# Easquel/WaveDM

Hardware: AMD Instinct MI355X
Metric: restored images/sec, raindrop 64x64 patches, 100-step DDIM (higher is better)
Workload: dtype bf16; 1 GPU; raindrop_wavelet 64x64 (256x256 px crops), batch 64/GPU, 100 DDIM steps, DWT + UNet x100 + IDWT (BASELINE.json configs[1]); global_batch=64, ddim_steps=100, parallelism=image-sharded x1, outputs_finite=True

## Files before the change

wavedm_amd/csrc/blocks.hip:

```cpp
#include <stdarg.h>

#include <algorithm>
#include <cmath>

#include <atomic>
#include <mutex>
#include "common.h"
#include "gn_inline.h"

namespace wdm {

static thread_local char g_err[512] = "";
void set_error(const char* fmt, ...) {
    va_list ap;
    va_start(ap, fmt);
    vsnprintf(g_err, sizeof(g_err), fmt, ap);
    va_end(ap);
}
const char* get_error() { return g_err; }

void* Arena::alloc(size_t bytes) {
    bytes = align_up(bytes ? bytes : 1, 256);
    for (size_t i = 0; i < free_.size(); ++i) {
        if (free_[i].len >= bytes) {
// ... 16 lines not shown
        if (used_[i].off == off) {
            Blk b = used_[i];
            used_.erase(used_.begin() + i);
            auto it = std::lower_bound(free_.begin(), free_.end(), b, [](const Blk& a, const Blk& c) { return a.off < c.off; });
            it = free_.insert(it, b);
            if (it + 1 != free_.end() && it->off + it->len == (it + 1)->off) { it->len += (it + 1)->len; free_.erase(it + 1); }
            if (it != free_.begin() && (it - 1)->off + (it - 1)->len == it->off) { (it - 1)->len += it->len; free_.erase(it); }
            return;
        }
    }
}

int alloc_tens(Ctx& c, int C, int H, int W, Tens* t) {
    *t = Tens();
    t->C = C; t->H = H; t->W = W; t->xs = C;
    t->p = c.ar->alloc((size_t)c.B * H * W * C * dsize(c.dtype));
    if (!t->p) WDM_FAIL(WDM_ENOMEM, "workspace too small (tensor %dx%dx%dx%d)", c.B, H, W, C);
    return WDM_OK;
}
void free_tens(Ctx& c, Tens& t) {
    c.ar->free(t.p);
    if (t.stats) c.ar->free(t.stats);
    if (t.nrm) c.ar->free(t.nrm);
    t.p = nullptr; t.stats = nullptr; t.gst = nullptr; t.nslab = 0; t.nrm = nullptr; t.nrm_for = nullptr;
}

static int alloc_f32(Ctx& c, size_t n, float** p) {
    *p = (float*)c.ar->alloc(n * sizeof(float));
    if (!*p) WDM_FAIL(WDM_ENOMEM, "workspace too small (%zu floats)", n);
    return WDM_OK;
}

static std::atomic<const EnvCfg*> g_env{nullptr};
static std::mutex g_env_mu;
void env_cfg_refresh() {
    EnvCfg* c = new EnvCfg();
    auto flag = [](const char* name, int dflt) { const char* e = getenv(name); return e ? (e[0] == '0' ? 0 : 1) : dflt; };
    auto num = [](const char* name, int dflt) { const char* e = getenv(name); return e ? atoi(e) : dflt; };
    c->conv_dma = flag("WDM_CONV_DMA", 1); c->gemm = flag("WDM_GEMM", 1); c->bn256 = num("WDM_BN256", 1);
    c->gn_tile = num("WDM_GN_TILE", 2); c->gn_inline = flag("WDM_GN_INLINE", 1); c->attn_fused = num("WDM_ATTN_FUSED", 3); c->attn_fold = num("WDM_ATTN_FOLD", 1);
    c->up4 = flag("WDM_UP4", 1); c->attn_sm = flag("WDM_ATTN_SM", 1); c->attn_stream = flag("WDM_ATTN_STREAM", 1); c->wgrad_bg = num("WDM_WGRAD_BG", 0);
    std::lock_guard<std::mutex> lk(g_env_mu);
    g_env.store(c, std::memory_order_release);
}
const EnvCfg& env_cfg() {
    const EnvCfg* c = g_env.load(std::memory_order_acquire);
    if (!c) {
        {
            std::lock_guard<std::mutex> lk(g_env_mu);
            c = g_env.load(std::memory_order_acquire);
        }
        if (!c) { env_cfg_refresh(); c = g_env.load(std::memory_order_acquire); }
    }
    return *c;
}

bool conv_up4_eligible(int dtype, int H, int W, int cin, int cout) {
    return env_cfg().up4 && (is_h16(dtype) || dtype == WDM_F32X3) && ((H % 16 == 0 && W % 16 == 0) || (H == 8 && W == 8)) && cin % 32 == 0 && cout % 8 == 0 && cout >= 128;
}

int launch_conv(const ConvArgs& a, int mode, int dtype, hipStream_t s) {
    return dtype == WDM_BF16 ? launch_conv_bf16(a, mode, s) : dtype == WDM_F16 ? launch_conv_f16(a, mode, s) : dtype == WDM_F32X3 ? launch_conv_f32x3(a, mode, s) : launch_conv_f32(a, mode, s);
}
ConvArgs gemm_args(int B, int H, int W, const void* x, int xs, int K, const void* w, int ws, long long w_img, int rows, int cout, void* y, int y_mode, size_t es,
                   float alpha) {
    ConvArgs a{};
    a.x0 = x; a.C0 = K; a.xs0 = xs;
    a.B = B; a.Hin = a.Hout = H; a.Win = a.Wout = W;
    a.Cin = K; a.Cout = cout;
    a.w = w; a.w_img_stride = w_img; a.w_row_stride = ws; a.w_rows = rows;
    a.w_bytes = (unsigned)((size_t)rows * ws * es);
    a.alpha = alpha;
    a.y = y; a.y_mode = y_mode; a.y_s = cout;
    return a;
}
int run_conv(Ctx& c, const ConvW& w, int mode, const ConvReq& r, Tens* out, ConvArgs* defer) {
    const Tens& x0 = *r.x0;
    const Tens* x1 = r.x1;
    const int Cin = x0.C + (x1 ? x1->C : 0);
    if (Cin != w.cin) WDM_FAIL(WDM_EINVAL, "conv: input has %d channels, weights expect %d", Cin, w.cin);
    if (x1 && (x1->H != x0.H || x1->W != x0.W)) WDM_FAIL(WDM_EINVAL, "conv: concat inputs differ in size");
    int Ho = x0.H, Wo = x0.W;
    if (mode == MODE_S2) { Ho = x0.H / 2; Wo = x0.W / 2; }
    if (mode == MODE_UPS) { Ho = x0.H * 2; Wo = x0.W * 2; }
    void* y = r.y_ext;
    const int y_mode = r.y_ext ? r.y_mode : Y_NHWC;
    if (!r.y_ext) {
        WDM_TRY(alloc_tens(c, w.cout, Ho, Wo, out));
        y = out->p;
    }
    ConvArgs a{};
    a.x0 = x0.p; a.x1 = x1 ? x1->p : nullptr;
    a.C0 = x0.C; a.C1 = x1 ? x1->C : 0;
    a.xs0 = x0.xs; a.xs1 = x1 ? x1->xs : 0;
    a.B = c.B; a.Hin = x0.H; a.Win = x0.W; a.Hout = Ho; a.Wout = Wo;
    a.Cin = Cin; a.Cout = w.cout;
    a.w = w.w; a.w_tap_stride = (long long)w.rows_pad * w.cin; a.w_img_stride = 0; a.w_row_stride = w.cin; a.w_rows = w.rows_pad;
    a.w_bytes = (unsigned)((size_t)w.k * w.k * w.rows_pad * w.cin * dsize(c.dtype));
    a.w_sm = ((mode == MODE_S1 || (mode == MODE_S2 && is_h16(c.dtype))) && w.k == 3) ? w.w_sm : nullptr;
    a.bias = w.b; a.alpha = 1.0f;
    a.pro = (r.scale || r.gn_inl) ? 1 : 0; a.scale = r.scale; a.shift = r.shift;
    if (r.gn_inl) {
        if (x1 || !x0.gst || r.scale || r.gn_inl->c != Cin) WDM_FAIL(WDM_EINVAL, "conv: in-prologue GroupNorm needs a single input with group partials");
        a.gin = x0.gst; a.gin_nslab = x0.nslab; a.gn_gamma = r.gn_inl->g; a.gn_beta = r.gn_inl->b; a.gn_eps = 1e-6f;
    }
    a.temb = r.temb; a.temb_ld = r.temb_ld; a.temb_per_image = r.temb_per_image;
    a.res = r.res ? r.res->p : nullptr; a.res_s = r.res ? r.res->xs : 0;
    a.y = y; a.y_mode = y_mode; a.y_s = w.cout;
    if (mode == MODE_UPS && w.w_up4 && !x1 && !r.scale && !r.temb && !r.res && !r.shortcut && y_mode == Y_NHWC && conv_up4_eligible(c.dtype, x0.H, x0.W, Cin, w.cout)) {
        mode = MODE_UP4;
        a.Hout = x0.H; a.Wout = x0.W;
        a.w = w.w_up4;
        a.w_bytes = (unsigned)((size_t)16 * w.rows_pad * w.cin * dsize(c.dtype));
    }
    if (r.shortcut) {
        a.sx0 = r.sx0->p; a.sx1 = r.sx1 ? r.sx1->p : nullptr;
        a.sC0 = r.sx0->C; a.sC1 = r.sx1 ? r.sx1->C : 0; a.sxs0 = r.sx0->xs; a.sxs1 = r.sx1 ? r.sx1->xs : 0;
        a.sw = r.shortcut->w; a.sw_row_stride = r.shortcut->cin; a.sw_rows = r.shortcut->rows_pad;
        a.sw_bytes = (unsigned)((size_t)r.shortcut->rows_pad * r.shortcut->cin * dsize(c.dtype));
        a.sbias = r.shortcut->b;
    }
    if (r.stats && !r.y_ext && w.cout % 8 == 0) {
        int nslab = 0, yn_ok = 0;
        ConvArgs q = a;
        q.query_nslab = &nslab; q.query_yn = &yn_ok;
        WDM_TRY(launch_conv(q, mode, c.dtype, c.s));
        out->nslab = nslab;
        if (r.on && yn_ok && env_cfg().gn_tile && r.on->c == w.cout) {
            out->nrm = c.ar->alloc((size_t)c.B * Ho * Wo * w.cout * dsize(c.dtype));
            if (!out->nrm) WDM_FAIL(WDM_ENOMEM, "workspace too small (normalised copy)");
            out->nrm_for = r.on->g; out->nrm_silu = r.on_silu;
            a.yn = out->nrm; a.on_gamma = r.on->g; a.on_beta = r.on->b; a.on_eps = 1e-6f; a.on_silu = r.on_silu;
        }
        const bool want_gst = is_h16(c.dtype) && env_cfg().gn_inline && gn_inline_shape_ok(w.cout, nslab);
        const size_t sb = gn_stats_bytes(c.B, nslab, w.cout);
        out->stats = (float*)c.ar->alloc(sb + (want_gst ? (size_t)c.B * nslab * 96 * sizeof(float) : 0));
        if (!out->stats) WDM_FAIL(WDM_ENOMEM, "workspace too small (GroupNorm statistics)");
        a.stats = out->stats; a.stats_nslab = nslab;
        if (want_gst) { out->gst = (float*)((char*)out->stats + sb); a.gst = out->gst; }
    }
    if (c.dry) return WDM_OK;
    if (defer) { *defer = a; return WDM_OK; }
    return launch_conv(a, mode, c.dtype, c.s);
}

static int gn_partials_of(Ctx& c, const Tens& x, float** st, int* ns, float** tmp) {
    *tmp = nullptr;
    if (x.stats) { *st = x.stats; *ns = x.nslab; return WDM_OK; }
    *ns = gn_default_nslab(x.H * x.W);
    *tmp = (float*)c.ar->alloc(gn_stats_bytes(c.B, *ns, x.C));
    if (!*tmp) WDM_FAIL(WDM_ENOMEM, "workspace too small (GroupNorm statistics)");
    *st = *tmp;
    if (!c.dry) WDM_TRY(k_gn_partial(x, c.B, *tmp, *ns, c.dtype, c.s));
    return WDM_OK;
}

int run_gn(Ctx& c, const NormW& nw, const Tens& x0, const Tens* x1, int for_silu_conv, float** scale, float** shift) {
    const int C = x0.C + (x1 ? x1->C : 0);
    WDM_TRY(alloc_f32(c, (size_t)c.B * C, scale));
    WDM_TRY(alloc_f32(c, (size_t)c.B * C, shift));
    float *st0 = nullptr, *st1 = nullptr, *tmp0 = nullptr, *tmp1 = nullptr;
    int ns0 = 0, ns1 = 0;
// ... 24 lines not shown
        int rc = WDM_OK;
        if (!c.dry) rc = k_gn_finalize_apply(c.B, x0, x1, st0, ns0, st1, ns1, nw, 1e-6f, silu, out->p, c.dtype, c.s);
        if (tmp0) c.ar->free(tmp0);
        if (tmp1) c.ar->free(tmp1);
        return rc;
    }
    float *sc, *sh;
    WDM_TRY(run_gn(c, nw, x0, x1, 0, &sc, &sh));
    WDM_TRY(alloc_tens(c, C, x0.H, x0.W, out));
    if (!c.dry) {
        WDM_TRY(k_gn_apply(x0, c.B, sc, sh, C, out->p, C, 0, silu, c.dtype, c.s));
        if (x1) WDM_TRY(k_gn_apply(*x1, c.B, sc + x0.C, sh + x0.C, C, out->p, C, x0.C, silu, c.dtype, c.s));
    }
    c.ar->free(sc); c.ar->free(sh);
    return WDM_OK;
}
static int materialize_gn_silu(Ctx& c, const NormW& nw, const Tens& x0, const Tens* x1, Tens* out) { return materialize_gn(c, nw, x0, x1, 1, out); }

static bool gn_inline_ok(const Ctx& c, const Tens& x0, const Tens* x1, int cout) {
    return env_cfg().gn_inline && env_cfg().conv_dma && is_h16(c.dtype) && !x1 && x0.gst != nullptr && gn_inline_shape_ok(x0.C, x0.nslab) && x0.H % 16 == 0 &&
           x0.W % 16 == 0 && cout >= 128;
}

int run_resblock(Ctx& c, const ResW& w, const Tens& x0, const Tens* x1, Tens* out, const NormW* next_n, int next_silu) {
    const int Cin = x0.C + (x1 ? x1->C : 0);
    if (Cin != w.cin) WDM_FAIL(WDM_EINVAL, "resblock: input has %d channels, block expects %d", Cin, w.cin);
    if (!w.has_nin && x1) WDM_FAIL(WDM_EINVAL, "resblock: identity shortcut cannot take a concat input");
    const bool pass = x0.H * x0.W <= GN_PASS_MAX_HW;
    ConvReq r1{.x0 = &x0, .x1 = x1, .temb = w.temb, .temb_ld = w.temb_ld, .temb_per_image = w.temb_per_image, .stats = true,
               .on = pass || env_cfg().gn_tile >= 2 ? &w.n2 : nullptr, .on_silu = 1};
    Tens a1, t1;
    float *sc1 = nullptr, *sh1 = nullptr;
    if (pass) {
        WDM_TRY(materialize_gn_silu(c, w.n1, x0, x1, &a1));
        r1.x0 = &a1; r1.x1 = nullptr;
    } else if (gn_inline_ok(c, x0, x1, w.cout)) {
        r1.gn_inl = &w.n1;
    } else {
        WDM_TRY(run_gn(c, w.n1, x0, x1, 1, &sc1, &sh1));
        r1.scale = sc1; r1.shift = sh1;
    }
    WDM_TRY(run_conv(c, w.c1, MODE_S1, r1, &t1));
    free_tens(c, a1);
    c.ar->free(sc1); c.ar->free(sh1);
    const bool pre2 = !pass && t1.nrm != nullptr && t1.nrm_for == w.n2.g && t1.nrm_silu == 1;
    const bool fuse_nin = w.has_nin && env_cfg().conv_dma && (!pass || (x0.H == 8 && x0.W == 8 && is_h16(c.dtype))) &&
                          (is_h16(c.dtype) || (c.dtype == WDM_F32X3 && x0.H % 16 == 0 && x0.W % 16 == 0)) &&
                          conv_can_fuse_shortcut(x0.H, x0.W, w.cout, w.cout, x0.C, x1 ? x1->C : 0);
    ConvReq r2{.x0 = &t1, .stats = true, .on = next_n, .on_silu = next_silu};
    Tens sct;
    if (fuse_nin) {
        r2.shortcut = &w.nin; r2.sx0 = &x0; r2.sx1 = x1;
    } else if (w.has_nin) {
        WDM_TRY(run_conv(c, w.nin, MODE_P1, {.x0 = &x0, .x1 = x1}, &sct));
        r2.res = &sct;
    } else {
        r2.res = &x0;
    }
    Tens a2;
    float *sc2 = nullptr, *sh2 = nullptr;
    if (pass || pre2) {
        WDM_TRY(materialize_gn_silu(c, w.n2, t1, nullptr, &a2));
        r2.x0 = &a2;
    } else if (gn_inline_ok(c, t1, nullptr, w.cout)) {
        r2.gn_inl = &w.n2;
    } else {
        WDM_TRY(run_gn(c, w.n2, t1, nullptr, 1, &sc2, &sh2));
        r2.scale = sc2; r2.shift = sh2;
    }
    WDM_TRY(run_conv(c, w.c2, MODE_S1, r2, out));
    free_tens(c, a2);
    c.ar->free(sc2); c.ar->free(sh2);
// ... 162 lines not shown
```

wavedm_amd/csrc/common.h:

```cpp
#pragma once
#include <hip/hip_runtime.h>
#include <stdint.h>
#include <stdio.h>
#include <string>
#include <vector>

#include "../../include/wavedm.h"
#include "conv_kernel.h"
#include "dropout.h"
#include "model_layout.h"

namespace wdm {

void set_error(const char* fmt, ...);
#define WDM_FAIL(code, ...)        \
    do {                           \
        wdm::set_error(__VA_ARGS__); \
        return (code);             \
    } while (0)
#define WDM_HIP(expr)                                                                        \
    do {                                                                                     \
        hipError_t e__ = (expr);                                                             \
        if (e__ != hipSuccess) WDM_FAIL(WDM_EHIP, "%s failed: %s", #expr, hipGetErrorString(e__)); \
    } while (0)
// ... 27 lines not shown
    bool failed() const { return failed_; }
    bool is_dry() const { return base_ == nullptr; }

   private:
    struct Blk { size_t off, len; };
    char* base_;
    size_t cap_;
    size_t peak_ = 0;
    bool failed_ = false;
    std::vector<Blk> free_;
    std::vector<Blk> used_;
};

struct Tens {
    void* p = nullptr;
    int C = 0, H = 0, W = 0;
    int xs = 0;
    float* stats = nullptr;
    int nslab = 0;
    float* gst = nullptr;
    void* nrm = nullptr;
    const float* nrm_for = nullptr;
    int nrm_silu = 0;
};

struct Ctx {
    hipStream_t s;
    int dtype;
    int B;
    Arena* ar;
    bool dry;
};

struct ConvW {
    const void* w = nullptr;
    const void* w_up4 = nullptr;
    const void* w_sm = nullptr;
    const float* b = nullptr;
    int cin = 0, cout = 0, k = 1, rows_pad = 0;
};
struct NormW {
    const float* g = nullptr;
    const float* b = nullptr;
    int c = 0;
};
constexpr int GN_PASS_MAX_HW = 64;
// ... 87 lines not shown
    int q_ld = 0, k_ld = 0, v_ld = 0;
    int v_tok = 0;
    const void* qw = nullptr; const float* qbias = nullptr; int qw_ld = 0; size_t qw_bytes = 0;
    int bdiag = 0;
    int qw_slab = 0;
};
int launch_attn_fused(const AttnOperands& in, void* o, int B, int C, hipStream_t s, const float* vbias = nullptr, const ConvArgs* proj = nullptr, int dtype = WDM_BF16);
bool attn_stream_eligible(int dtype, int N, int C);
int launch_attn_stream(const AttnOperands& in, void* o, int B, int N, int C, hipStream_t s, const float* vbias = nullptr, int dtype = WDM_BF16);
int k_attn_fold(const float* wq, const float* bq, const float* wk, const float* wv, const float* bv, const float* wp, const float* bp, int C, float* M, float* cq, float* Wvp,
                float* bvp, hipStream_t s);

struct EnvCfg {
    int conv_dma = 1;
    int gemm = 1;
    int bn256 = 1;
    int gn_tile = 2;
    int gn_inline = 1;
    int attn_fold = 1;
    int attn_fused = 3;
    int attn_sm = 1;
    int attn_stream = 1;
    int up4 = 1;
    int wgrad_bg = 0;
};
const EnvCfg& env_cfg();
void env_cfg_refresh();

int launch_conv(const ConvArgs& a, int mode, int dtype, hipStream_t s);
ConvArgs gemm_args(int B, int H, int W, const void* x, int xs, int K, const void* w, int ws, long long w_img, int rows, int cout, void* y, int y_mode, size_t es,
                   float alpha = 1.f);

struct ConvReq {
    const Tens* x0 = nullptr;
    const Tens* x1 = nullptr;
    const float* scale = nullptr;
    const float* shift = nullptr;
    const NormW* gn_inl = nullptr;
    const float* temb = nullptr;
    int temb_ld = 0;
    int temb_per_image = 0;
    const Tens* res = nullptr;
    int y_mode = Y_NHWC;
    void* y_ext = nullptr;
    bool stats = false;
    const ConvW* shortcut = nullptr;
    const Tens* sx0 = nullptr;
    const Tens* sx1 = nullptr;
    const NormW* on = nullptr;
    int on_silu = 0;
};
int run_conv(Ctx& c, const ConvW& w, int mode, const ConvReq& r, Tens* out, ConvArgs* defer = nullptr);
int run_gn(Ctx& c, const NormW& nw, const Tens& x0, const Tens* x1, int for_silu_conv, float** scale, float** shift);
int run_resblock(Ctx& c, const ResW& w, const Tens& x0, const Tens* x1, Tens* out, const NormW* next_n = nullptr, int next_silu = 0);
int run_attn(Ctx& c, const AttnW& w, const Tens& x, Tens* out);
int attn_tokens_check(int H, int W);
int alloc_tens(Ctx& c, int C, int H, int W, Tens* t);
void free_tens(Ctx& c, Tens& t);

int conv_dgrad(Ctx& c, int mode, const float* w_oihw, int cin, int cout, const Tens& dy, int H, int W, void* dx, bool accumulate, const void* wd_prepacked = nullptr);
size_t conv_dgrad_packed_bytes(int cin, int cout, int k, int dtype);
int k_pack_conv_both(const float* w_oihw, int cout, int cin, int k, void* dst_fwd, int rows_total, void* dst_dgrad, int dtype, hipStream_t s);
struct PackDesc { const float* w; void* dstf; void* dstd; int cout, cin, rows_total, rows_d, kpad, gx, blk0; };
struct PackBatch { static constexpr int MAX = 12; PackDesc d[MAX]; int n; };
int k_pack_conv_both_batch(const PackDesc* descs, int n, int k, int dtype, hipStream_t s);
int conv_wgrad(Ctx& c, int mode, const Tens& x0, const Tens* x1, const Tens& dy, int cout, float* dw, bool accumulate, float* db = nullptr, float* dtemb = nullptr,
               int dtemb_ld = 0);
int colsum(Ctx& c, const Tens& dy, float* out, bool per_image, bool accumulate, int out_ld = 0);
int gn_act_backward(Ctx& c, const NormW& nw, const Tens& x0, const Tens* x1, const float* mean_rstd, const Tens& dy, int silu, void* dx0, bool acc0, void* dx1,
                    bool acc1, float* dgamma, float* dbeta, bool acc_param, const Dropout* drop = nullptr);
int k_adam_ema(float* P, const float* G, float* M, float* V, float* E, long long n, int64_t step, float lr, double beta1, double beta2, float eps, float weight_decay,
               float ema_mu, hipStream_t s);
int k_optim_ema(int rule, float* P, const float* G, float* S0, float* S1, float* S2, float* E, long long n, int64_t step, double lr, double beta1, double beta2,
                double eps, double weight_decay, double ema_mu, hipStream_t s);

}

// ... 4 lines not shown
```

wavedm_amd/csrc/conv_dispatch.inc:

```
#include <stdlib.h>

#include <atomic>

#include "common.h"
#include "conv_kernel.h"
#include "gn_inline.h"
#ifndef WDM_DTYPE_NAME
#define WDM_DTYPE_NAME (sizeof(WDM_T) == 2 ? "bf16" : "f32")
#endif

#ifndef WDM_H16_NAME
#define WDM_H16_NAME "bf16"
#endif

namespace wdm {

static int ensure_max_lds(const void* kern, int bytes, std::atomic<unsigned>& devs) {
    int dev = 0;
    WDM_HIP(hipGetDevice(&dev));
    const unsigned bit = 1u << (dev & 31);
    if (!(devs.load(std::memory_order_acquire) & bit)) {
        WDM_HIP(hipFuncSetAttribute(kern, hipFuncAttributeMaxDynamicSharedMemorySize, bytes));
        devs.fetch_or(bit, std::memory_order_release);
    }
// ... 12 lines not shown

static int set_extents(ConvArgs& a, double rows, double es, const char* who) {
    const double b0 = rows * a.xs0 * es, b1 = rows * a.xs1 * es;
    if (b0 >= 4294901760.0 || b1 >= 4294901760.0) WDM_FAIL(WDM_EINVAL, "%s: input tensor of %.0f bytes exceeds the 4 GB buffer-offset range", who, b0 > b1 ? b0 : b1);
    a.x0_bytes = (unsigned)b0;
    a.x1_bytes = a.x1 ? (unsigned)b1 : 0u;
    if (a.w_bytes == 0) WDM_FAIL(WDM_EINVAL, "%s: w_bytes not set", who);
    return WDM_OK;
}
static int set_shortcut_extents(ConvArgs& a, double es, int kstep, const char* who) {
    if (!a.sx0) return WDM_OK;
    if (a.sC0 % kstep || (a.sC0 + a.sC1) % kstep || a.Hin != a.Hout || a.sw_bytes == 0) WDM_FAIL(WDM_EINVAL, "%s: shortcut operand unsupported", who);
    const double s0 = (double)a.B * a.Hout * a.Wout * a.sxs0 * es, s1 = (double)a.B * a.Hout * a.Wout * a.sxs1 * es;
    if (s0 >= 4294901760.0 || s1 >= 4294901760.0) WDM_FAIL(WDM_EINVAL, "%s: shortcut tensor exceeds the 4 GB buffer-offset range", who);
    a.sx0_bytes = (unsigned)s0;
    a.sx1_bytes = a.sx1 ? (unsigned)s1 : 0u;
    return WDM_OK;
}
static int check_stats(ConvArgs& a, int nslab, bool yn_ok, const char* who, bool* done) {
    *done = false;
    if (a.query_nslab) { *a.query_nslab = nslab; if (a.query_yn) *a.query_yn = yn_ok ? 1 : 0; *done = true; return WDM_OK; }
    if (a.stats && (a.stats_nslab != nslab || a.Cout % 8 || (a.y_mode != Y_NHWC && a.y_mode != Y_NHWC_F32)))
        WDM_FAIL(WDM_EINVAL, "%s: inconsistent GroupNorm-statistics request (nslab %d vs %d)", who, a.stats_nslab, nslab);
    if (a.yn && !(yn_ok && a.stats && a.on_gamma && a.on_beta)) WDM_FAIL(WDM_EINVAL, "%s: in-tile GroupNorm of the output unsupported for this launch", who);
    return WDM_OK;
}
static void use_slab_major(ConvArgs& a) {
    if (a.w_sm) { a.w = a.w_sm; a.w_tap_stride = (long long)a.w_rows * 32; a.w_row_stride = 32; a.w_slab_stride = 9 * a.w_rows * 32; }
}
struct Work { double flops, bytes; };
static Work conv_work(const ConvArgs& a, double taps, double es, double in_pix, double out_pix) {
    const double sK = a.sx0 ? (double)(a.sC0 + a.sC1) : 0.0;
    Work w;
    w.flops = 2.0 * out_pix * a.Cout * (taps * a.Cin + sK);
    w.bytes = in_pix * a.Cin * es + out_pix * sK * es + a.Cout * (taps * a.Cin + sK) * es * (a.w_img_stride ? a.B : 1) + out_pix * a.Cout * (a.y_mode >= Y_NCHW_F32 ? 4.0 : es) +
              (a.res ? out_pix * a.Cout * es : 0.0) + (a.yn ? out_pix * a.Cout * es : 0.0);
    return w;
}
template <class K>
static int launch_named(K kern, int grid, int threads, int lds, hipStream_t s, const ConvArgs& a, std::atomic<unsigned>& devs, const char* name, Work w) {
    WDM_TRY(ensure_max_lds((const void*)kern, lds, devs));
    const bool prof = prof_enabled();
    if (prof) prof_begin(s, name, w.flops, w.bytes);
    hipLaunchKernelGGL(kern, dim3(grid), dim3(threads), lds, s, a);
    if (prof) prof_end(s);
    WDM_HIP(hipGetLastError());
    return WDM_OK;
}
#define WDM_NAME(buf, ...) char buf[112]; snprintf(buf, sizeof(buf), __VA_ARGS__)

template <int MODE, int TH, int TW, int NI, int WAVES_M, int WAVES_N, int WM, int WN, int KSUB = 4>
static int launch_cfg(const ConvArgs& a0, hipStream_t s) {
    using C = ConvCfg<WDM_T, MODE, TH, TW, NI, WAVES_M, WAVES_N, WM, WN, KSUB>;
    ConvArgs a = a0;
    if (a.Hout % TH || a.Wout % TW) WDM_FAIL(WDM_EINVAL, "conv: %dx%d output not divisible by the %dx%d tile", a.Hout, a.Wout, TH, TW);
    if (NI > 1 && (a.Hout != TH || a.Wout != TW)) WDM_FAIL(WDM_EINVAL, "conv: multi-image tile needs %dx%d output", TH, TW);
    if (a.Cin % C::BK || a.C0 % C::BK) WDM_FAIL(WDM_EINVAL, "conv: Cin=%d / C0=%d must be multiples of %d", a.Cin, a.C0, C::BK);
    WDM_TRY(set_extents(a, a.m_valid ? (double)a.m_valid : (double)a.B * a.Hin * a.Win, sizeof(WDM_T), "conv"));
// ... 264 lines not shown
    int grid;
    plain_grid(a, &grid);
    WDM_NAME(name, "gemmx3_1x1_t16x16x1_bn128_f32x3|%dx%d %d->%d", a.Hout, a.Wout, a.Cin, a.Cout);
    static std::atomic<unsigned> devs{0};
    return launch_named(conv_gemmx3_kernel, grid, C::NTHREADS, C::LDS_BYTES, s, a, devs, name, conv_work(a, 1.0, 4.0, (double)a.B * a.Hin * a.Win, (double)a.B * a.Hout * a.Wout));
}
#endif

int WDM_LAUNCH_NAME(const ConvArgs& a, int mode, hipStream_t s) {
    const bool t16 = (a.Hout % 16 == 0) && (a.Wout % 16 == 0);
    const bool t8 = (a.Hout % 8 == 0) && (a.Wout % 8 == 0);
    const bool img8 = (a.Hout == 8 && a.Wout == 8);
    const bool bn16 = a.Cout <= 16;
    const bool shared_w = a.w_img_stride == 0;
    const bool dma = env_cfg().conv_dma != 0, gemm = env_cfg().gemm != 0;
    (void)dma; (void)gemm; (void)shared_w;
    if (!t8) WDM_FAIL(WDM_EINVAL, "conv: output %dx%d must be a multiple of 8", a.Hout, a.Wout);
    if ((a.y_mode == Y_NHWC || a.y_mode == Y_NHWC_F32) && a.Cout % 8 == 0) {
        const double rows = mode == MODE_UP4 ? 4.0 * a.B * a.Hout * a.Wout : a.m_valid ? (double)a.m_valid : (double)a.B * a.Hout * a.Wout;
        const double yb = rows * a.y_s * (a.y_mode == Y_NHWC ? (double)sizeof(WDM_T) : 4.0), rb = a.res ? rows * a.res_s * (double)sizeof(WDM_T) : 0.0;
        if (yb >= 4026531840.0 || rb >= 4026531840.0)
            WDM_FAIL(WDM_EINVAL, "conv: output / residual tensor of %.0f bytes exceeds the 32-bit buffer-offset range", yb > rb ? yb : rb);
    }
    if (a.query_yn) *a.query_yn = 0;
    if (a.yn && !a.query_nslab) {
        int ok = 0, ns = 0;
        ConvArgs q = a;
        q.query_nslab = &ns; q.query_yn = &ok;
        WDM_TRY(WDM_LAUNCH_NAME(q, mode, s));
        if (!ok) WDM_FAIL(WDM_EINVAL, "conv: in-tile GroupNorm of the output requested for a conv whose kernel cannot write it");
    }
    if (a.gst && (a.Cout % 32 || !gn_inline_shape_ok(a.Cout, a.stats_nslab) || !a.stats)) WDM_FAIL(WDM_EINVAL, "conv: group partials requested for Cout = %d", a.Cout);
    if (a.gin) {
#ifdef WDM_HAS_GEMM
        const bool dma_ok = mode == MODE_S1 && t16 && !bn16 && a.Cout >= 128 && dma && a.x1 == nullptr && shared_w && gn_inline_shape_ok(a.Cin, a.gin_nslab) && a.gn_gamma && a.gn_beta;
#else
        const bool dma_ok = false;
#endif
        if (!dma_ok) WDM_FAIL(WDM_EINVAL, "conv: in-prologue GroupNorm requested for a conv the LDS-DMA kernels do not take");
    }
#if defined(WDM_HAS_DMAX3)
    constexpr bool sc_ok_t = true;
#else
    constexpr bool sc_ok_t = sizeof(WDM_T) == 2;
#endif
    if (a.sx0 && !(mode == MODE_S1 && sc_ok_t && dma && conv_can_fuse_shortcut(a.Hout, a.Wout, a.Cin, a.Cout, a.sC0, a.sC1)))
// ... 76 lines not shown
```

wavedm_amd/csrc/conv_kernel.h:

```cpp
#pragma once
#include <hip/hip_runtime.h>
#include <stdint.h>

#ifndef WDM_ABL
#define WDM_ABL 0
#endif
#ifndef WDM_STORE_AUX
#define WDM_STORE_AUX 2
#endif

namespace wdm {

typedef __attribute__((ext_vector_type(4))) float f32x4;
typedef __attribute__((ext_vector_type(8))) __bf16 bf16x8;
typedef unsigned short bf16_raw;

enum { MODE_S1 = 0, MODE_S2 = 1, MODE_UPS = 2, MODE_P1 = 3, MODE_UP4 = 4 };
enum { Y_NHWC = 0, Y_NCHW = 1, Y_NCHW_F32 = 2, Y_NHWC_F32 = 3 };

struct ConvArgs {
    const void* x0;
    const void* x1;
    int C0, C1;
    int xs0, xs1;
// ... 303 lines not shown
#pragma unroll
    for (int jp = 0; jp < WN; jp += NJ) {
        float* const ep = ep0 + (jp / NJ) * keep_stride;
        if (jp == 0) { WDM_ETS(1); if (entry_barrier) __syncthreads(); WDM_ETS(2); }
        else { __builtin_amdgcn_fence(__ATOMIC_RELEASE, "wavefront"); __builtin_amdgcn_wave_barrier(); }
        if (active) write_pass(ep, jp);
        __builtin_amdgcn_fence(__ATOMIC_RELEASE, "wavefront");
        __builtin_amdgcn_wave_barrier();
        if (jp == 0) { asm volatile("s_waitcnt lgkmcnt(0)" ::: "memory"); WDM_ETS(3); }
        if (!active) continue;
        const int ncol0 = n0 + (wave_n * WN + jp) * 16;
        if (vec_ok) {
            const int c8 = (lane % LPR) * 8, lp = lane / LPR;
            const int n = ncol0 + c8;
            const bool ncol = n < a.Cout;
            constexpr unsigned OOBV = 0xFFFF0000u;
            const int es_y = a.y_mode == Y_NHWC ? ES : 4;
            const int lane_pix = !a.up4 ? (lp / TW) * a.Wout + (lp % TW) : ((lp / TW) * 2) * (2 * a.Wout) + (lp % TW) * 2;
            const unsigned vo_y = ncol ? (unsigned)((lane_pix * a.y_s + n) * es_y) : OOBV;
            const unsigned vo_r = ncol ? (unsigned)((lane_pix * a.res_s + n) * ES) : OOBV;
            float bias8[8];
#pragma unroll
            for (int e = 0; e < 8; ++e) bias8[e] = add8[jp / NJ][e];
            const bool do_stats = a.stats != nullptr && !pre_applied;
            constexpr int NIT = (EROWS + RPI - 1) / RPI;
            constexpr bool RAGGED = EROWS % RPI != 0;
            int so_pix[NIT];
            bool img_ok[NIT];
            int img_it[NIT];
#pragma unroll
            for (int it = 0; it < NIT; ++it) {
                const int mu = wave_m * EROWS + it * RPI;
                const int img_u = mu / (TH * TW), rru = mu % (TH * TW);
                const int oyu = oy0 + rru / TW, oxu = ox0 + rru % TW;
                const int img_g = img0 + img_u;
                img_it[it] = img_g;
                img_ok[it] = img_g < a.B;
                so_pix[it] = !a.up4 ? (img_g * a.Hout + oyu) * a.Wout + oxu
                                    : (img_g * (2 * a.Hout) + 2 * oyu + (phase >> 1)) * (2 * a.Wout) + 2 * oxu + (phase & 1);
            }
            uint4 resv[VEC == 8 ? NIT : 1];
            if (VEC == 8 && a.res != nullptr) {
#pragma unroll
                for (int it = 0; it < NIT; ++it) {
                    unsigned vo = vo_r;
                    if (a.m_valid != 0 && so_pix[it] + lane_pix >= a.m_valid) vo = OOBV;
                    if (RAGGED && it * RPI + lp >= EROWS) vo = OOBV;
// ... 25 lines not shown
                }
                if (!pre_applied && !TEMB_IN_ADD && a.temb != nullptr && ncol) {
                    const float* tp = a.temb + (long long)(a.temb_per_image ? img_it[it] : 0) * a.temb_ld + n;
                    const float4 t0 = *(const float4*)tp, t1 = *(const float4*)(tp + 4);
                    v[0] += t0.x; v[1] += t0.y; v[2] += t0.z; v[3] += t0.w; v[4] += t1.x; v[5] += t1.y; v[6] += t1.z; v[7] += t1.w;
                }
                if (a.res != nullptr) {
                    float rf[8];
                    if (VEC == 8) TI<T>::unpack(resv[it], rf);
                    else {
                        const int so = (int)((unsigned)so_pix[it] * (unsigned)a.res_s * (unsigned)ES);
                        TI<T>::unpack(__builtin_bit_cast(uint4, __builtin_amdgcn_raw_buffer_load_b128(r_res, (int)vor, so, 0)), rf);
                        TI<T>::unpack(__builtin_bit_cast(uint4, __builtin_amdgcn_raw_buffer_load_b128(r_res, (int)vor + 16, so, 0)), rf + 4);
                    }
#pragma unroll
                    for (int e = 0; e < 8; ++e) v[e] += rf[e];
                }
                float vr[8];
                const unsigned vst = voy == OOBV ? OOBV : voy + (unsigned)so_pix[it] * (unsigned)a.y_s * (unsigned)es_y;
                typedef unsigned u32x4 __attribute__((ext_vector_type(4)));
                if (a.y_mode == Y_NHWC && VEC == 8) {
                    const uint4 pk = TI<T>::pack(v);
                    TI<T>::unpack(pk, vr);
                    if (!(WDM_EABL & 1)) __builtin_amdgcn_raw_buffer_store_b128(__builtin_bit_cast(u32x4, pk), r_y, (int)vst, 0, WDM_STORE_AUX);
                } else {
#pragma unroll
                    for (int e = 0; e < 8; ++e) vr[e] = v[e];
                    if (!(WDM_EABL & 1)) {
                        __builtin_amdgcn_raw_buffer_store_b128(__builtin_bit_cast(u32x4, make_float4(v[0], v[1], v[2], v[3])), r_y, (int)vst, 0, WDM_STORE_AUX);
                        __builtin_amdgcn_raw_buffer_store_b128(__builtin_bit_cast(u32x4, make_float4(v[4], v[5], v[6], v[7])), r_y, (int)vst + 16, 0, WDM_STORE_AUX);
                    }
                }
                if (do_stats && row_ok) {
                    *(float4*)(ep + rloc * ESTR + c8) = make_float4(vr[0], vr[1], vr[2], vr[3]);
                    *(float4*)(ep + rloc * ESTR + c8 + 4) = make_float4(vr[4], vr[5], vr[6], vr[7]);
                }
            }
            WDM_ETS(4);
            if (jp == 0) hook();
            if (do_stats) {
                __builtin_amdgcn_fence(__ATOMIC_RELEASE, "wavefront");
                __builtin_amdgcn_wave_barrier();
                constexpr int SROWS = conv_stat_rows(TH, TW, EROWS);
                constexpr int PARTS = 64 / ECOLS;
                constexpr int RPP = EROWS / PARTS;
                static_assert(SROWS % RPP == 0 && EROWS % SROWS == 0, "statistics slab geometry");
                const int col = lane % ECOLS, part = lane / ECOLS;
                const int r0 = part * RPP;
                const int srow = (r0 / SROWS) * SROWS;
                const float K = ep[srow * ESTR + col];
                float s1 = 0.f, s2 = 0.f;
// ... 8 lines not shown
                    for (int r = 0; r < CH; ++r) { const float d = ep[(r0 + ch * CH + r) * ESTR + col] - K; c1 += d; c2 = __builtin_fmaf(d, d, c2); }
                    cs1[ch] = c1; cs2[ch] = c2;
                    if (ch == 0) { s1 = c1; s2 = c2; } else { s1 += c1; s2 += c2; }
                }
                if (CANON && SROWS / RPP > 1) {
                    constexpr int GPS = SROWS / RPP;
                    const int base = (part / GPS) * GPS;
#pragma unroll
                    for (int pg = 0; pg < GPS; ++pg)
#pragma unroll
                        for (int ch = 0; ch < NCH; ++ch) {
                            const float v1 = __shfl(cs1[ch], col + ECOLS * (base + pg)), v2 = __shfl(cs2[ch], col + ECOLS * (base + pg));
                            if (pg == 0 && ch == 0) { s1 = v1; s2 = v2; } else { s1 += v1; s2 += v2; }
                        }
                } else {
#pragma unroll
                    for (int off = ECOLS; off < ECOLS * (SROWS / RPP); off <<= 1) { s1 += __shfl_xor(s1, off); s2 += __shfl_xor(s2, off); }
                }
                const int m0 = wave_m * EROWS + srow;
                const int img_g = img0 + m0 / (TH * TW);
                constexpr int SPT = (TH * TW) / SROWS;
                const int slab = tile_in_img * SPT + (m0 % (TH * TW)) / SROWS + (a.up4 ? phase * (a.stats_nslab >> 2) : 0);
                const int nn = ncol0 + col;
                if ((r0 % SROWS) == 0 && nn < a.Cout && img_g < a.B)
                    ((float4*)a.stats)[((long long)img_g * a.stats_nslab + slab) * a.Cout + nn] = make_float4(K, s1, s2, (float)SROWS);
                if (keep_tab != nullptr && (r0 % SROWS) == 0 && nn < a.Cout)
                    keep_tab[((m0 / (TH * TW)) * SPT + (m0 % (TH * TW)) / SROWS) * keep_bn + (nn - n0)] = make_float4(K, s1, s2, (float)SROWS);
                if (a.gst != nullptr) {
                    const int gs = a.Cout >> 5;
                    const float Kg = __shfl(K, lane & ~(gs - 1));
                    const float d = K - Kg, nr = (float)SROWS;
                    float g1 = __builtin_fmaf(nr, d, s1);
                    float g2 = __builtin_fmaf(nr * d, d, __builtin_fmaf(2.0f * d, s1, s2));
                    for (int off = 1; off < gs; off <<= 1) { g1 += __shfl_xor(g1, off); g2 += __shfl_xor(g2, off); }
                    if ((r0 % SROWS) == 0 && (lane & (gs - 1)) == 0 && nn < a.Cout && img_g < a.B) {
                        float* q = a.gst + (((long long)img_g * a.stats_nslab + slab) * 32 + nn / gs) * 3;
                        q[0] = Kg; q[1] = g1; q[2] = g2;
                    }
                }
            }
        } else {
#pragma unroll 1
            for (int it = 0; it < (EROWS + 63) / 64; ++it) {
                const int rloc = it * 64 + lane;
                if (rloc >= EROWS) continue;
                const int m = wave_m * EROWS + rloc;
                const int img = m / (TH * TW), rr = m % (TH * TW);
// ... 80 lines not shown
                if (a.sbias != nullptr) { const float4 c = *(const float4*)(a.sbias + n); ad.x += c.x; ad.y += c.y; ad.z += c.z; ad.w += c.w; }
                if (a.temb != nullptr) { const float4 c = *(const float4*)(a.temb + trow * a.temb_ld + n); ad.x += c.x; ad.y += c.y; ad.z += c.z; ad.w += c.w; }
            }
            const int wr = wr0 + (((j * 2 + (quad >> 1)) ^ (px & 7)) << 4);
#pragma unroll
            for (int i = 0; i < 4; ++i) {
                const f32x4 v = acc[i][jp + j];
                float f0 = __builtin_fmaf(v[0], a.alpha, ad.x), f1 = __builtin_fmaf(v[1], a.alpha, ad.y), f2 = __builtin_fmaf(v[2], a.alpha, ad.z), f3 = __builtin_fmaf(v[3], a.alpha, ad.w);
                if (has_res) {
                    const uint2 rr = *(const uint2*)(tp + wr + i * (16 * ROWB));
                    float r0, r1, r2, r3;
                    TI<T>::unpack2(rr.x, r0, r1); TI<T>::unpack2(rr.y, r2, r3);
                    f0 += r0; f1 += r1; f2 += r2; f3 += r3;
                }
                uint2 pk;
                pk.x = TI<T>::pack2(f0, f1);
                pk.y = TI<T>::pack2(f2, f3);
                *(uint2*)(tp + wr + i * (16 * ROWB)) = pk;
            }
        }
    }
    __builtin_amdgcn_fence(__ATOMIC_RELEASE, "wavefront");
    __builtin_amdgcn_wave_barrier();
    {
        constexpr unsigned OOBV = 0xFFFF0000u;
        const long long out_rows = a.up4 ? (long long)a.B * 4 * a.Hout * a.Wout : (long long)a.B * a.Hout * a.Wout;
        const __amdgpu_buffer_rsrc_t r_y = __builtin_amdgcn_make_buffer_rsrc(a.y, 0, (int)(unsigned)(out_rows * a.y_s * 2), 0x00020000);
        const int c8 = (lane & 7) * 8, lp = lane >> 3;
        const int n = ncol0 + c8;
        const int lane_pix = !a.up4 ? lp : lp * 2;
        const unsigned vo_y = n < a.Cout ? (unsigned)((lane_pix * a.y_s + n) * 2) : OOBV;
        const int rd = lp * ROWB + (((lane & 7) ^ lp) << 4);
        uint4 tl[8];
#pragma unroll
        for (int it = 0; it < 8; ++it) tl[it] = *(const uint4*)(tp + rd + it * (8 * ROWB));
#pragma unroll
        for (int it = 0; it < 8; ++it) {
            const int mu = wave_m * EROWS + it * 8;
            const int img_u = mu / (TH * TW), rru = mu % (TH * TW);
            const int oyu = oy0 + rru / TW, oxu = ox0 + rru % TW;
            const int img_g = img0 + img_u;
            if (img_g >= a.B) continue;
            const int so_pix = !a.up4 ? (img_g * a.Hout + oyu) * a.Wout + oxu
                                      : (img_g * (2 * a.Hout) + 2 * oyu + (phase >> 1)) * (2 * a.Wout) + 2 * oxu + (phase & 1);
            const unsigned vst = vo_y == OOBV ? OOBV : vo_y + (unsigned)so_pix * (unsigned)a.y_s * 2u;
            typedef unsigned u32x4 __attribute__((ext_vector_type(4)));
            const u32x4 pk = (it & 1) ? u32x4{tl[it].z, tl[it].w, tl[it].x, tl[it].y} : u32x4{tl[it].x, tl[it].y, tl[it].z, tl[it].w};
            if (!(WDM_EABL & 1)) __builtin_amdgcn_raw_buffer_store_b128(pk, r_y, (int)vst, 0, WDM_STORE_AUX);
        }
    }
    if (call_hook) hook();
    if (a.stats != nullptr) {
        const int col = lane, u = col >> 3, e = col & 7;
        int va[2][8];
#pragma unroll
        for (int h = 0; h < 2; ++h)
#pragma unroll
            for (int k = 0; k < 8; ++k) va[h][k] = ((u ^ k) << 4) | ((((e >> 2) ^ h)) << 3) | ((e & 3) << 1);
        auto val = [&](int r) __attribute__((always_inline)) {
            return TI<T>::raw16_to_f32(*(const unsigned short*)(tp + r * ROWB + va[(r >> 3) & 1][r & 7]));
        };
        const float K = val(0);
        float s1 = 0.f, s2 = 0.f;
#pragma unroll
        for (int ch = 0; ch < 4; ++ch) {
            float c1 = 0.f, c2 = 0.f;
#pragma unroll
            for (int r = 0; r < 16; ++r) { const float d = val(ch * 16 + r) - K; c1 += d; c2 = __builtin_fmaf(d, d, c2); }
            if (ch == 0) { s1 = c1; s2 = c2; } else { s1 += c1; s2 += c2; }
            __builtin_amdgcn_sched_barrier(0);
        }
        const int m0 = wave_m * EROWS;
        const int img_g = img0 + m0 / (TH * TW);
        constexpr int SPT = (TH * TW) / 64;
        const int slab = tile_in_img * SPT + (m0 % (TH * TW)) / 64 + (a.up4 ? phase * (a.stats_nslab >> 2) : 0);
        const int nn = ncol0 + col;
        if (nn < a.Cout && img_g < a.B) ((float4*)a.stats)[((long long)img_g * a.stats_nslab + slab) * a.Cout + nn] = make_float4(K, s1, s2, 64.f);
        if (keep_tab != nullptr && nn < a.Cout) keep_tab[((m0 / (TH * TW)) * SPT + (m0 % (TH * TW)) / 64) * keep_bn + (nn - n0)] = make_float4(K, s1, s2, 64.f);
        if (a.gst != nullptr) {
            const int gs = a.Cout >> 5;
            const float Kg = __shfl(K, lane & ~(gs - 1));
            const float d = K - Kg, nr = 64.f;
            float g1 = __builtin_fmaf(nr, d, s1);
            float g2 = __builtin_fmaf(nr * d, d, __builtin_fmaf(2.0f * d, s1, s2));
            for (int off = 1; off < gs; off <<= 1) { g1 += __shfl_xor(g1, off); g2 += __shfl_xor(g2, off); }
            if ((lane & (gs - 1)) == 0 && nn < a.Cout && img_g < a.B) {
                float* q = a.gst + (((long long)img_g * a.stats_nslab + slab) * 32 + nn / gs) * 3;
                q[0] = Kg; q[1] = g1; q[2] = g2;
            }
        }
    }
}

template <typename T, int TH, int TW, int WM, int WN, int NJ_ = 0, class Hook = EpiNoHook, bool CANON = false, int PACK = 0, class AT = ConvArgs>
__device__ __forceinline__ void conv_epilogue(const AT& a, f32x4 (&acc)[WM][WN], char* smem, bool active, int wave, int lane, int wave_m,
                                              int wave_n, int img0, int oy0, int ox0, int n0, int tile_in_img, int phase = 0, Hook hook = Hook(),
                                              bool entry_barrier = true, float4* keep_tab = nullptr, int keep_bn = 0) {
    if (WDM_EABL & 2) { float t = 0.f; for (int i = 0; i < WM; ++i) for (int j = 0; j < WN; ++j) t += acc[i][j][0] + acc[i][j][1] + acc[i][j][2] + acc[i][j][3]; if (t == 123.456f) ((float*)a.y)[0] = t; return; }
    constexpr int NJ = NJ_ ? NJ_ : ((WN >= 2) ? 2 : 1);
    constexpr int ESTR = 16 * NJ + 4;
// ... 328 lines not shown
```

wavedm_amd/csrc/unet.hip:

```cpp
#include <string.h>

#include <map>
#include <mutex>
#include <string>

#include "common.h"

namespace wdm {
const char* get_error();
}
using namespace wdm;

namespace {

enum ParamKind { PK_CONV, PK_F32 };

struct ParamSlot {
    ParamKind kind = PK_F32;
    size_t off = 0;
    int rows_total = 0;
    int row_off = 0;
    bool zero_tail = true;
    int cin_dst = 0;
    size_t sm_off = 0;
// ... 252 lines not shown
            }
            hs.push_back(o);
        }
        if (l != nres - 1) {
            Tens o;
            WDM_TRY(run_conv(c, cw(L.down_ds[l]), MODE_S2, {.x0 = &hs.back(), .stats = true}, &o));
            hs.push_back(o);
        }
    }
    Tens m1, m2;
    const NormW mid_n = aw(mid_attn).n;
    WDM_TRY(run_resblock(c, rw(mid1, temb_all, n_t), hs.back(), nullptr, &m1, &mid_n, 0));
    WDM_TRY(run_attn(c, aw(mid_attn), m1, &m2));
    free_tens(c, m1);
    WDM_TRY(run_resblock(c, rw(mid2, temb_all, n_t), m2, nullptr, &h));
    free_tens(c, m2);
    for (int l = nres - 1; l >= 0; --l) {
        for (int b = 0; b <= nrb; ++b) {
            Tens skip = hs.back();
            hs.pop_back();
            Tens o;
            NormW nn;
            if (!up_attn[l].empty()) nn = aw(up_attn[l][b]).n;
            WDM_TRY(run_resblock(c, rw(up_res[l][b], temb_all, n_t), h, &skip, &o, up_attn[l].empty() ? nullptr : &nn, 0));
            free_tens(c, h);
            free_tens(c, skip);
            h = o;
            if (!up_attn[l].empty()) {
                Tens o2;
                WDM_TRY(run_attn(c, aw(up_attn[l][b]), h, &o2));
                free_tens(c, h);
                h = o2;
            }
        }
        if (l != 0) {
            Tens o;
            WDM_TRY(run_conv(c, cw(L.up_us[l]), MODE_UPS, {.x0 = &h, .stats = true}, &o));
            free_tens(c, h);
            h = o;
        }
    }
    {
        float *sc, *sh;
        WDM_TRY(run_gn(c, nw(L.norm_out), h, nullptr, 1, &sc, &sh));
        Tens dummy;
        WDM_TRY(run_conv(c, cw(L.conv_out), MODE_S1, {.x0 = &h, .scale = sc, .shift = sh, .y_mode = Y_NCHW_F32, .y_ext = eps_out}, &dummy));
        c.ar->free(sc); c.ar->free(sh);
// ... 135 lines not shown
```

Measured before the change: 134.5 img/s.

## Skip raw conv1 output store when only normalised copy is consumed

In resblocks, the first conv's raw output is only read through its fused GroupNorm+SiLU normalised copy. The conv can now skip writing the raw tensor and the global GroupNorm stats, keeping only the in-tile stats table used for the yn copy. It also drops statistics for resblock outputs that feed an upsample conv directly. Mode 2, the default, still allocates the skipped buffers as 'held' so the arena layout stays the same. This trades extra plumbing and a new null-output path against lower HBM write traffic.

```diff
diff --git a/wavedm_amd/csrc/blocks.hip b/wavedm_amd/csrc/blocks.hip
--- a/wavedm_amd/csrc/blocks.hip
+++ b/wavedm_amd/csrc/blocks.hip
@@ -62,6 +62,8 @@
     c.ar->free(t.p);
     if (t.stats) c.ar->free(t.stats);
     if (t.nrm) c.ar->free(t.nrm);
+    c.ar->free(t.held[0]); c.ar->free(t.held[1]);
+    t.held[0] = t.held[1] = nullptr;
     t.p = nullptr; t.stats = nullptr; t.gst = nullptr; t.nslab = 0; t.nrm = nullptr; t.nrm_for = nullptr;
 }
 
@@ -80,6 +82,7 @@
     c->conv_dma = flag("WDM_CONV_DMA", 1); c->gemm = flag("WDM_GEMM", 1); c->bn256 = num("WDM_BN256", 1);
     c->gn_tile = num("WDM_GN_TILE", 2); c->gn_inline = flag("WDM_GN_INLINE", 1); c->attn_fused = num("WDM_ATTN_FUSED", 3); c->attn_fold = num("WDM_ATTN_FOLD", 1);
     c->up4 = flag("WDM_UP4", 1); c->attn_sm = flag("WDM_ATTN_SM", 1); c->attn_stream = flag("WDM_ATTN_STREAM", 1); c->wgrad_bg = num("WDM_WGRAD_BG", 0);
+    c->conv1_yn_only = num("WDM_CONV1_YN_ONLY", 2);
     std::lock_guard<std::mutex> lk(g_env_mu);
     g_env.store(c, std::memory_order_release);
 }
@@ -123,12 +126,7 @@
     int Ho = x0.H, Wo = x0.W;
     if (mode == MODE_S2) { Ho = x0.H / 2; Wo = x0.W / 2; }
     if (mode == MODE_UPS) { Ho = x0.H * 2; Wo = x0.W * 2; }
-    void* y = r.y_ext;
     const int y_mode = r.y_ext ? r.y_mode : Y_NHWC;
-    if (!r.y_ext) {
-        WDM_TRY(alloc_tens(c, w.cout, Ho, Wo, out));
-        y = out->p;
-    }
     ConvArgs a{};
     a.x0 = x0.p; a.x1 = x1 ? x1->p : nullptr;
     a.C0 = x0.C; a.C1 = x1 ? x1->C : 0;
@@ -146,7 +144,7 @@
     }
     a.temb = r.temb; a.temb_ld = r.temb_ld; a.temb_per_image = r.temb_per_image;
     a.res = r.res ? r.res->p : nullptr; a.res_s = r.res ? r.res->xs : 0;
-    a.y = y; a.y_mode = y_mode; a.y_s = w.cout;
+    a.y = r.y_ext; a.y_mode = y_mode; a.y_s = w.cout;
     if (mode == MODE_UPS && w.w_up4 && !x1 && !r.scale && !r.temb && !r.res && !r.shortcut && y_mode == Y_NHWC && conv_up4_eligible(c.dtype, x0.H, x0.W, Cin, w.cout)) {
         mode = MODE_UP4;
         a.Hout = x0.H; a.Wout = x0.W;
@@ -160,24 +158,40 @@
         a.sw_bytes = (unsigned)((size_t)r.shortcut->rows_pad * r.shortcut->cin * dsize(c.dtype));
         a.sbias = r.shortcut->b;
     }
-    if (r.stats && !r.y_ext && w.cout % 8 == 0) {
-        int nslab = 0, yn_ok = 0;
+    const bool want_stats = r.stats && !r.y_ext && w.cout % 8 == 0;
+    int nslab = 0, yn_ok = 0;
+    if (want_stats) {
         ConvArgs q = a;
         q.query_nslab = &nslab; q.query_yn = &yn_ok;
         WDM_TRY(launch_conv(q, mode, c.dtype, c.s));
-        out->nslab = nslab;
-        if (r.on && yn_ok && env_cfg().gn_tile && r.on->c == w.cout) {
-            out->nrm = c.ar->alloc((size_t)c.B * Ho * Wo * w.cout * dsize(c.dtype));
-            if (!out->nrm) WDM_FAIL(WDM_ENOMEM, "workspace too small (normalised copy)");
-            out->nrm_for = r.on->g; out->nrm_silu = r.on_silu;
-            a.yn = out->nrm; a.on_gamma = r.on->g; a.on_beta = r.on->b; a.on_eps = 1e-6f; a.on_silu = r.on_silu;
-        }
+    }
+    const bool yn = want_stats && r.on && yn_ok && env_cfg().gn_tile && r.on->c == w.cout;
+    const bool yn_only = yn && r.raw_unused && env_cfg().conv1_yn_only;
+    const bool hold = yn_only && env_cfg().conv1_yn_only >= 2;
+    if (!r.y_ext) {
+        if (yn_only) {
+            *out = Tens(); out->C = w.cout; out->H = Ho; out->W = Wo; out->xs = w.cout;
+            if (hold && !(out->held[0] = c.ar->alloc((size_t)c.B * Ho * Wo * w.cout * dsize(c.dtype)))) WDM_FAIL(WDM_ENOMEM, "workspace too small (tensor %dx%dx%dx%d)", c.B, Ho, Wo, w.cout);
+        } else WDM_TRY(alloc_tens(c, w.cout, Ho, Wo, out));
+        a.y = out->p;
+    }
+    if (yn) {
+        out->nrm = c.ar->alloc((size_t)c.B * Ho * Wo * w.cout * dsize(c.dtype));
+        if (!out->nrm) WDM_FAIL(WDM_ENOMEM, "workspace too small (normalised copy)");
+        out->nrm_for = r.on->g; out->nrm_silu = r.on_silu;
+        a.yn = out->nrm; a.on_gamma = r.on->g; a.on_beta = r.on->b; a.on_eps = 1e-6f; a.on_silu = r.on_silu;
+    }
+    if (want_stats && (!yn_only || hold)) {
         const bool want_gst = is_h16(c.dtype) && env_cfg().gn_inline && gn_inline_shape_ok(w.cout, nslab);
         const size_t sb = gn_stats_bytes(c.B, nslab, w.cout);
-        out->stats = (float*)c.ar->alloc(sb + (want_gst ? (size_t)c.B * nslab * 96 * sizeof(float) : 0));
-        if (!out->stats) WDM_FAIL(WDM_ENOMEM, "workspace too small (GroupNorm statistics)");
-        a.stats = out->stats; a.stats_nslab = nslab;
-        if (want_gst) { out->gst = (float*)((char*)out->stats + sb); a.gst = out->gst; }
+        float* st = (float*)c.ar->alloc(sb + (want_gst ? (size_t)c.B * nslab * 96 * sizeof(float) : 0));
+        if (!st) WDM_FAIL(WDM_ENOMEM, "workspace too small (GroupNorm statistics)");
+        if (yn_only) out->held[1] = st;
+        else {
+            out->nslab = nslab; out->stats = st;
+            a.stats = st; a.stats_nslab = nslab;
+            if (want_gst) { out->gst = (float*)((char*)st + sb); a.gst = out->gst; }
+        }
     }
     if (c.dry) return WDM_OK;
     if (defer) { *defer = a; return WDM_OK; }
@@ -248,13 +262,13 @@
            x0.W % 16 == 0 && cout >= 128;
 }
 
-int run_resblock(Ctx& c, const ResW& w, const Tens& x0, const Tens* x1, Tens* out, const NormW* next_n, int next_silu) {
+int run_resblock(Ctx& c, const ResW& w, const Tens& x0, const Tens* x1, Tens* out, const NormW* next_n, int next_silu, bool out_stats) {
     const int Cin = x0.C + (x1 ? x1->C : 0);
     if (Cin != w.cin) WDM_FAIL(WDM_EINVAL, "resblock: input has %d channels, block expects %d", Cin, w.cin);
     if (!w.has_nin && x1) WDM_FAIL(WDM_EINVAL, "resblock: identity shortcut cannot take a concat input");
     const bool pass = x0.H * x0.W <= GN_PASS_MAX_HW;
     ConvReq r1{.x0 = &x0, .x1 = x1, .temb = w.temb, .temb_ld = w.temb_ld, .temb_per_image = w.temb_per_image, .stats = true,
-               .on = pass || env_cfg().gn_tile >= 2 ? &w.n2 : nullptr, .on_silu = 1};
+               .on = pass || env_cfg().gn_tile >= 2 ? &w.n2 : nullptr, .on_silu = 1, .raw_unused = true};
     Tens a1, t1;
     float *sc1 = nullptr, *sh1 = nullptr;
     if (pass) {
@@ -273,7 +287,7 @@
     const bool fuse_nin = w.has_nin && env_cfg().conv_dma && (!pass || (x0.H == 8 && x0.W == 8 && is_h16(c.dtype))) &&
                           (is_h16(c.dtype) || (c.dtype == WDM_F32X3 && x0.H % 16 == 0 && x0.W % 16 == 0)) &&
                           conv_can_fuse_shortcut(x0.H, x0.W, w.cout, w.cout, x0.C, x1 ? x1->C : 0);
-    ConvReq r2{.x0 = &t1, .stats = true, .on = next_n, .on_silu = next_silu};
+    ConvReq r2{.x0 = &t1, .stats = out_stats, .on = next_n, .on_silu = next_silu};
     Tens sct;
     if (fuse_nin) {
         r2.shortcut = &w.nin; r2.sx0 = &x0; r2.sx1 = x1;
diff --git a/wavedm_amd/csrc/common.h b/wavedm_amd/csrc/common.h
--- a/wavedm_amd/csrc/common.h
+++ b/wavedm_amd/csrc/common.h
@@ -73,6 +73,7 @@
     void* nrm = nullptr;
     const float* nrm_for = nullptr;
     int nrm_silu = 0;
+    void* held[2] = {nullptr, nullptr};
 };
 
 struct Ctx {
@@ -206,6 +207,7 @@
     int attn_sm = 1;
     int attn_stream = 1;
     int up4 = 1;
+    int conv1_yn_only = 2;
     int wgrad_bg = 0;
 };
 const EnvCfg& env_cfg();
@@ -233,10 +235,11 @@
     const Tens* sx1 = nullptr;
     const NormW* on = nullptr;
     int on_silu = 0;
+    bool raw_unused = false;
 };
 int run_conv(Ctx& c, const ConvW& w, int mode, const ConvReq& r, Tens* out, ConvArgs* defer = nullptr);
 int run_gn(Ctx& c, const NormW& nw, const Tens& x0, const Tens* x1, int for_silu_conv, float** scale, float** shift);
-int run_resblock(Ctx& c, const ResW& w, const Tens& x0, const Tens* x1, Tens* out, const NormW* next_n = nullptr, int next_silu = 0);
+int run_resblock(Ctx& c, const ResW& w, const Tens& x0, const Tens* x1, Tens* out, const NormW* next_n = nullptr, int next_silu = 0, bool out_stats = true);
 int run_attn(Ctx& c, const AttnW& w, const Tens& x, Tens* out);
 int attn_tokens_check(int H, int W);
 int alloc_tens(Ctx& c, int C, int H, int W, Tens* t);
diff --git a/wavedm_amd/csrc/conv_dispatch.inc b/wavedm_amd/csrc/conv_dispatch.inc
--- a/wavedm_amd/csrc/conv_dispatch.inc
+++ b/wavedm_amd/csrc/conv_dispatch.inc
@@ -58,7 +58,7 @@
     if (a.query_nslab) { *a.query_nslab = nslab; if (a.query_yn) *a.query_yn = yn_ok ? 1 : 0; *done = true; return WDM_OK; }
     if (a.stats && (a.stats_nslab != nslab || a.Cout % 8 || (a.y_mode != Y_NHWC && a.y_mode != Y_NHWC_F32)))
         WDM_FAIL(WDM_EINVAL, "%s: inconsistent GroupNorm-statistics request (nslab %d vs %d)", who, a.stats_nslab, nslab);
-    if (a.yn && !(yn_ok && a.stats && a.on_gamma && a.on_beta)) WDM_FAIL(WDM_EINVAL, "%s: in-tile GroupNorm of the output unsupported for this launch", who);
+    if (a.yn && !(yn_ok && a.on_gamma && a.on_beta)) WDM_FAIL(WDM_EINVAL, "%s: in-tile GroupNorm of the output unsupported for this launch", who);
     return WDM_OK;
 }
 static void use_slab_major(ConvArgs& a) {
@@ -69,7 +69,7 @@
     const double sK = a.sx0 ? (double)(a.sC0 + a.sC1) : 0.0;
     Work w;
     w.flops = 2.0 * out_pix * a.Cout * (taps * a.Cin + sK);
-    w.bytes = in_pix * a.Cin * es + out_pix * sK * es + a.Cout * (taps * a.Cin + sK) * es * (a.w_img_stride ? a.B : 1) + out_pix * a.Cout * (a.y_mode >= Y_NCHW_F32 ? 4.0 : es) +
+    w.bytes = in_pix * a.Cin * es + out_pix * sK * es + a.Cout * (taps * a.Cin + sK) * es * (a.w_img_stride ? a.B : 1) + (a.y ? out_pix * a.Cout * (a.y_mode >= Y_NCHW_F32 ? 4.0 : es) : 0.0) +
               (a.res ? out_pix * a.Cout * es : 0.0) + (a.yn ? out_pix * a.Cout * es : 0.0);
     return w;
 }
@@ -380,6 +380,7 @@
         if (yb >= 4026531840.0 || rb >= 4026531840.0)
             WDM_FAIL(WDM_EINVAL, "conv: output / residual tensor of %.0f bytes exceeds the 32-bit buffer-offset range", yb > rb ? yb : rb);
     }
+    if (!a.y && !a.yn && !a.query_nslab) WDM_FAIL(WDM_EINVAL, "conv: no output (y is null and no normalised copy is requested)");
     if (a.query_yn) *a.query_yn = 0;
     if (a.yn && !a.query_nslab) {
         int ok = 0, ns = 0;
diff --git a/wavedm_amd/csrc/conv_kernel.h b/wavedm_amd/csrc/conv_kernel.h
--- a/wavedm_amd/csrc/conv_kernel.h
+++ b/wavedm_amd/csrc/conv_kernel.h
@@ -349,7 +349,8 @@
             float bias8[8];
 #pragma unroll
             for (int e = 0; e < 8; ++e) bias8[e] = add8[jp / NJ][e];
-            const bool do_stats = a.stats != nullptr && !pre_applied;
+            const bool do_stats = (a.stats != nullptr || keep_tab != nullptr) && !pre_applied;
+            const bool st_y = keep_tab == nullptr || a.y != nullptr;
             constexpr int NIT = (EROWS + RPI - 1) / RPI;
             constexpr bool RAGGED = EROWS % RPI != 0;
             int so_pix[NIT];
@@ -421,11 +422,11 @@
                 if (a.y_mode == Y_NHWC && VEC == 8) {
                     const uint4 pk = TI<T>::pack(v);
                     TI<T>::unpack(pk, vr);
-                    if (!(WDM_EABL & 1)) __builtin_amdgcn_raw_buffer_store_b128(__builtin_bit_cast(u32x4, pk), r_y, (int)vst, 0, WDM_STORE_AUX);
+                    if (!(WDM_EABL & 1) && st_y) __builtin_amdgcn_raw_buffer_store_b128(__builtin_bit_cast(u32x4, pk), r_y, (int)vst, 0, WDM_STORE_AUX);
                 } else {
 #pragma unroll
                     for (int e = 0; e < 8; ++e) vr[e] = v[e];
-                    if (!(WDM_EABL & 1)) {
+                    if (!(WDM_EABL & 1) && st_y) {
                         __builtin_amdgcn_raw_buffer_store_b128(__builtin_bit_cast(u32x4, make_float4(v[0], v[1], v[2], v[3])), r_y, (int)vst, 0, WDM_STORE_AUX);
                         __builtin_amdgcn_raw_buffer_store_b128(__builtin_bit_cast(u32x4, make_float4(v[4], v[5], v[6], v[7])), r_y, (int)vst + 16, 0, WDM_STORE_AUX);
                     }
@@ -480,7 +481,7 @@
                 constexpr int SPT = (TH * TW) / SROWS;
                 const int slab = tile_in_img * SPT + (m0 % (TH * TW)) / SROWS + (a.up4 ? phase * (a.stats_nslab >> 2) : 0);
                 const int nn = ncol0 + col;
-                if ((r0 % SROWS) == 0 && nn < a.Cout && img_g < a.B)
+                if (a.stats != nullptr && (r0 % SROWS) == 0 && nn < a.Cout && img_g < a.B)
                     ((float4*)a.stats)[((long long)img_g * a.stats_nslab + slab) * a.Cout + nn] = make_float4(K, s1, s2, (float)SROWS);
                 if (keep_tab != nullptr && (r0 % SROWS) == 0 && nn < a.Cout)
                     keep_tab[((m0 / (TH * TW)) * SPT + (m0 % (TH * TW)) / SROWS) * keep_bn + (nn - n0)] = make_float4(K, s1, s2, (float)SROWS);
@@ -607,7 +608,7 @@
     }
     __builtin_amdgcn_fence(__ATOMIC_RELEASE, "wavefront");
     __builtin_amdgcn_wave_barrier();
-    {
+    if (keep_tab == nullptr || a.y != nullptr) {
         constexpr unsigned OOBV = 0xFFFF0000u;
         const long long out_rows = a.up4 ? (long long)a.B * 4 * a.Hout * a.Wout : (long long)a.B * a.Hout * a.Wout;
         const __amdgpu_buffer_rsrc_t r_y = __builtin_amdgcn_make_buffer_rsrc(a.y, 0, (int)(unsigned)(out_rows * a.y_s * 2), 0x00020000);
@@ -635,7 +636,7 @@
         }
     }
     if (call_hook) hook();
-    if (a.stats != nullptr) {
+    if (a.stats != nullptr || keep_tab != nullptr) {
         const int col = lane, u = col >> 3, e = col & 7;
         int va[2][8];
 #pragma unroll
@@ -660,7 +661,7 @@
         constexpr int SPT = (TH * TW) / 64;
         const int slab = tile_in_img * SPT + (m0 % (TH * TW)) / 64 + (a.up4 ? phase * (a.stats_nslab >> 2) : 0);
         const int nn = ncol0 + col;
-        if (nn < a.Cout && img_g < a.B) ((float4*)a.stats)[((long long)img_g * a.stats_nslab + slab) * a.Cout + nn] = make_float4(K, s1, s2, 64.f);
+        if (a.stats != nullptr && nn < a.Cout && img_g < a.B) ((float4*)a.stats)[((long long)img_g * a.stats_nslab + slab) * a.Cout + nn] = make_float4(K, s1, s2, 64.f);
         if (keep_tab != nullptr && nn < a.Cout) keep_tab[((m0 / (TH * TW)) * SPT + (m0 % (TH * TW)) / 64) * keep_bn + (nn - n0)] = make_float4(K, s1, s2, 64.f);
         if (a.gst != nullptr) {
             const int gs = a.Cout >> 5;
diff --git a/wavedm_amd/csrc/unet.hip b/wavedm_amd/csrc/unet.hip
--- a/wavedm_amd/csrc/unet.hip
+++ b/wavedm_amd/csrc/unet.hip
@@ -298,7 +298,8 @@
             Tens o;
             NormW nn;
             if (!up_attn[l].empty()) nn = aw(up_attn[l][b]).n;
-            WDM_TRY(run_resblock(c, rw(up_res[l][b], temb_all, n_t), h, &skip, &o, up_attn[l].empty() ? nullptr : &nn, 0));
+            const bool out_stats = !(b == nrb && l != 0 && up_attn[l].empty());
+            WDM_TRY(run_resblock(c, rw(up_res[l][b], temb_all, n_t), h, &skip, &o, up_attn[l].empty() ? nullptr : &nn, 0, out_stats));
             free_tens(c, h);
             free_tens(c, skip);
             h = o;
```

After: 134.9 img/s, median of 2. No clear change (+0.3%).
